# Voyager0587/yolov8-vit

Measured on AMD Instinct MI355X. Metric: images/sec end-to-end (640->224 detect+classify), higher is better.
Workload: dtype bf16; 1 GPU; YOLOv8n(nc=5)+ViT-B/16 end-to-end inference, 640x640, bf16 (BASELINE.json configs[1]); batch_per_gpu=32, global_batch=32, crops_per_image=4, parallelism=dp1, weights=random-init, seed 42

## Files before the change

### include/yv_hip.h

```cpp
#ifndef YV_HIP_H
#define YV_HIP_H

#include <stddef.h>
#include <stdint.h>

#ifdef __cplusplus
extern "C" {
#endif

#define YV_OK 0
#define YV_ERR_ARG (-1)
#define YV_ERR_LIMIT (-2)
#define YV_ERR_WORKSPACE (-3)
#define YV_ERR_LAUNCH (-4)

int yv_version(void);
const char* yv_error_string(int code);
int yv_device_is_gfx950(void);
int yv_set_option(const char* key, int value);
int yv_get_option(const char* key, int* value);

int yv_linear_mxfp8_q(const void* Aq, long long lda, const void* Ascale, long long a_rows_pad, const void* Wq, const void* Wscale,
                      long long w_rows_pad, const float* bias, int M, int N, int K, int flags, const int32_t* m_dev, int m_mul,
                      void* out_q, long long ldq, void* out_scales, long long out_rows_pad, void* stream);
// ... 102 lines not shown
    int ld;
    int c;
    int up;
} yv_view;

#define YV_EPI_BIAS 1
#define YV_EPI_SILU 2
#define YV_EPI_GELU 4
#define YV_EPI_RES_F32 8
#define YV_EPI_RES_BF16 16
#define YV_EPI_OUT_F32 32
#define YV_EPI_POSEMB 64
#define YV_EPI_SAVE_PRE 128
#define YV_EPI_GELU_BWD 256
#define YV_EPI_OUT_MXFP8 512

int yv_conv2d(const yv_view* in0, const yv_view* in1, int B, int Hout, int Wout, int ksize, int stride,
              const void* weight, const float* bias, int Cout, void* out, int out_ld, const void* res, int res_ld,
              int flags, void* stream);

int yv_conv2d_instance(int B, int Hout, int Wout, int ksize, int stride, int c0, int c1, int Cout, int out_ld, int res_ld,
                       int flags, size_t ws_bytes);

typedef struct yv_mx_view {
    const void* q;
    const void* s;
    int ld;
    int c;
    int up;
} yv_mx_view;

int yv_quant_mxfp8_map(const void* x, long long ldx, long long pixels, int C, void* q, long long ldq, void* scales,
                       void* stream);

int yv_conv2d_mxfp8(const yv_mx_view* in0, const yv_mx_view* in1, int B, int Hout, int Wout, int ksize, int stride,
                    const void* wq, const void* wscale, long long w_rows_pad, const float* bias, int Cout, void* out_bf16,
                    int out_ld, void* out_q, void* out_scales, int outq_ld, const void* res, int res_ld, int flags,
                    void* stream);
int yv_conv2d_mxfp8_instance(int B, int Hout, int Wout, int ksize, int stride, int Cin, int Cout);

int yv_c2f_fused(const void* x, long long ldx, int B, int H, int W, int c, int n, const void* w_cv1, const float* b_cv1,
                 const void* const* w_m, const float* const* b_m, const void* w_cv2, const float* b_cv2, void* out,
                 long long ldo, void* stream);
int yv_c2f_debug(void* buf);

int yv_conv2d_ws(const yv_view* in0, const yv_view* in1, int B, int Hout, int Wout, int ksize, int stride,
// ... 171 lines not shown
```

### yolov8-vit_amd/csrc/gemm.hip

```cpp
#include <string.h>
#include <type_traits>
#include <map>
#include <mutex>
#include "gemm_common.h"

using namespace yvgemm;

thread_local hipEvent_t yvgemm::t_time_start = nullptr, yvgemm::t_time_stop = nullptr;

namespace {

int g_opt_wgrad_split = 0;
int g_opt_wgrad_cap = 128;
int g_opt_variant = 1;
int g_opt_group_m = 8;
int g_opt_staged = 1;
int g_opt_p8 = 3;
std::mutex g_ws_mu;
std::map<void*, std::pair<void*, size_t>> g_ws;
static bool ws_lookup(void* stream, void** ws, size_t* bytes) {
    std::lock_guard<std::mutex> lk(g_ws_mu);
    auto it = g_ws.find(stream);
    if (it == g_ws.end()) return false;
    *ws = it->second.first; *bytes = it->second.second;
// ... 60 lines not shown
                float* o = (float*)g.out + orow * g.ldo + n;
                if (flags & YV_EPI_RES_F32) {
                    const float4 x = *(const float4*)o;
                    v[0] += x.x; v[1] += x.y; v[2] += x.z; v[3] += x.w;
                }
                *(float4*)o = make_float4(v[0], v[1], v[2], v[3]);
            } else {
                uint16_t* o = (uint16_t*)g.out + orow * g.ldo + n;
                *(uint2*)o = make_uint2(pack_bf16x2(v[0], v[1]), pack_bf16x2(v[2], v[3]));
                if constexpr (STATS) {
                    const uint32_t pk[2] = {pack_bf16x2(v[0], v[1]), pack_bf16x2(v[2], v[3])};
#pragma unroll
                    for (int q = 0; q < 4; ++q) {
                        const float f = bf16_to_f32((uint16_t)(q & 1 ? pk[q >> 1] >> 16 : pk[q >> 1] & 0xffff));
                        cs[i * 4 + q] += f; cq[i * 4 + q] += f * f;
                    }
                }
            }
        }
    }
}


template <int MF, bool STATS = false, bool PHASE = false >
__device__ __forceinline__ void epilogue_staged(const GemmArgs& g, f32x4 (&acc)[4][MF], int M, int m0, int n0,
                                                int wrow_m, int wrow_n, int lane, unsigned char* stage, float* cs = nullptr,
                                                float* cq = nullptr, int ph = 0) {
    const int flags = g.flags;
    const int fr = lane & 15, fq = lane >> 4;
    const int nb = n0 + wrow_n;
    float4 bv[4];
#pragma unroll
    for (int i = 0; i < 4; ++i) {
        const int n = nb + i * 16 + fq * 4;
        bv[i] = ((flags & YV_EPI_BIAS) && n < g.N) ? *(const float4*)(g.bias + n) : make_float4(0.f, 0.f, 0.f, 0.f);
    }
    auto value = [&](int i, int j, float* v, bool act = true) {
        v[0] = acc[i][j][0] + bv[i].x; v[1] = acc[i][j][1] + bv[i].y;
        v[2] = acc[i][j][2] + bv[i].z; v[3] = acc[i][j][3] + bv[i].w;
        if (!act) return;
        if (flags & YV_EPI_SILU) {
#pragma unroll
            for (int q = 0; q < 4; ++q) v[q] = silu_f(v[q]);
        }
        if (flags & YV_EPI_GELU) {
#pragma unroll
            for (int q = 0; q < 4; ++q) v[q] = gelu_f(v[q]);
        }
    };
    if (!(flags & (YV_EPI_OUT_F32 | YV_EPI_RES_F32))) {
        if (flags & YV_EPI_SAVE_PRE) {
#pragma unroll
            for (int j = 0; j < MF; ++j)
#pragma unroll
                for (int i = 0; i < 4; ++i) {
                    float v[4];
                    value(i, j, v, false);
                    const int row = j * 16 + fr, c16 = i * 2 + (fq >> 1);
                    *(uint2*)(stage + row * 128 + ((c16 ^ (row & 7)) << 4) + (fq & 1) * 8) =
                        make_uint2(pack_bf16x2(v[0], v[1]), pack_bf16x2(v[2], v[3]));
                }
#pragma unroll
            for (int it = 0; it < MF * 2; ++it) {
                const int row = it * 8 + (lane >> 3), ch = lane & 7;
                const int m = m0 + wrow_m + row, n = nb + ch * 8;
                const uint4 pk = *(const uint4*)(stage + row * 128 + ((ch ^ (row & 7)) << 4));
                if (m < M && n < g.N) *(uint4*)(g.aux + (long long)m * g.ldaux + n) = pk;
            }
        }
#pragma unroll
        for (int j = 0; j < MF; ++j)
#pragma unroll
            for (int i = 0; i < 4; ++i) {
                float v[4];
                value(i, j, v);
                const int row = j * 16 + fr, c16 = i * 2 + (fq >> 1);
                *(uint2*)(stage + row * 128 + ((c16 ^ (row & 7)) << 4) + (fq & 1) * 8) =
                    make_uint2(pack_bf16x2(v[0], v[1]), pack_bf16x2(v[2], v[3]));
            }
#pragma unroll
        for (int it = 0; it < MF * 2; ++it) {
            const int row = it * 8 + (lane >> 3), ch = lane & 7;
            const int m = m0 + wrow_m + row, n = nb + ch * 8;
            uint4 pk = *(const uint4*)(stage + row * 128 + ((ch ^ (row & 7)) << 4));
            if (m < M && n < g.N) {
                [[maybe_unused]] long long om = 0;
                if constexpr (PHASE) om = phase_row<true>(g, m, ph);
                if (flags & YV_EPI_RES_BF16) {
                    const uint4 rr = *(const uint4*)(g.res + (PHASE ? om : (long long)m) * g.ldres + n);
                    const uint32_t a[4] = {pk.x, pk.y, pk.z, pk.w}, b[4] = {rr.x, rr.y, rr.z, rr.w};
                    uint32_t o[4];
#pragma unroll
                    for (int q = 0; q < 4; ++q)
                        o[q] = pack_bf16x2(bf16_to_f32((uint16_t)(a[q] & 0xffff)) + bf16_to_f32((uint16_t)(b[q] & 0xffff)),
                                           bf16_to_f32((uint16_t)(a[q] >> 16)) + bf16_to_f32((uint16_t)(b[q] >> 16)));
                    pk = make_uint4(o[0], o[1], o[2], o[3]);
                }
                if (flags & YV_EPI_OUT_MXFP8) {
                    const uint32_t a[4] = {pk.x, pk.y, pk.z, pk.w};
                    float f[8];
#pragma unroll
                    for (int q = 0; q < 4; ++q) { f[2 * q] = bf16_to_f32((uint16_t)(a[q] & 0xffff)); f[2 * q + 1] = bf16_to_f32((uint16_t)(a[q] >> 16)); }
                    float amax = 0.f;
#pragma unroll
                    for (int q = 0; q < 8; ++q) amax = fmaxf(amax, fabsf(f[q]));
                    amax = fmaxf(amax, __shfl_xor(amax, 1, 64));
                    amax = fmaxf(amax, __shfl_xor(amax, 2, 64));
                    int e = -127;
                    if (amax > 0.f) {
                        int ex;
                        const float mant = frexpf(amax * (1.0f / 448.0f), &ex);
                        e = mant == 0.5f ? ex - 1 : ex;
                        e = e < -127 ? -127 : (e > 127 ? 127 : e);
                    }
                    const float inv = ldexpf(1.0f, -e);
                    int p0 = 0, p1 = 0;
                    p0 = __builtin_amdgcn_cvt_pk_fp8_f32(f[0] * inv, f[1] * inv, p0, false);
                    p0 = __builtin_amdgcn_cvt_pk_fp8_f32(f[2] * inv, f[3] * inv, p0, true);
                    p1 = __builtin_amdgcn_cvt_pk_fp8_f32(f[4] * inv, f[5] * inv, p1, false);
                    p1 = __builtin_amdgcn_cvt_pk_fp8_f32(f[6] * inv, f[7] * inv, p1, true);
                    *(uint2*)(g.mxq + (long long)m * g.ldmxq + n) = make_uint2((uint32_t)p0, (uint32_t)p1);
                    if ((ch & 3) == 0) {
                        const int bk = n >> 5;
                        g.mxs[((long long)(bk >> 2) * g.mx_rows + m) * 4 + (bk & 3)] = (uint8_t)(e + 127);
                    }
                    continue;
                }
                if (flags & YV_EPI_GELU_BWD) {
                    const uint4 uu = *(const uint4*)(g.aux + (long long)m * g.ldaux + n);
                    const uint32_t a[4] = {pk.x, pk.y, pk.z, pk.w}, b[4] = {uu.x, uu.y, uu.z, uu.w};
                    uint32_t o[4];
#pragma unroll
                    for (int q = 0; q < 4; ++q)
                        o[q] = pack_bf16x2(bf16_to_f32((uint16_t)(a[q] & 0xffff)) * gelu_grad_f(bf16_to_f32((uint16_t)(b[q] & 0xffff))),
                                           bf16_to_f32((uint16_t)(a[q] >> 16)) * gelu_grad_f(bf16_to_f32((uint16_t)(b[q] >> 16))));
                    pk = make_uint4(o[0], o[1], o[2], o[3]);
                }
                *(uint4*)((uint16_t*)g.out + (PHASE ? om : (long long)m) * g.ldo + n) = pk;
                if constexpr (STATS) {
                    const uint32_t a[4] = {pk.x, pk.y, pk.z, pk.w};
#pragma unroll
                    for (int q = 0; q < 8; ++q) {
                        const float f = bf16_to_f32((uint16_t)(q & 1 ? a[q >> 1] >> 16 : a[q >> 1] & 0xffff));
                        cs[q] += f; cq[q] += f * f;
                    }
                }
            }
        }
    } else {
#pragma unroll
        for (int half = 0; half < 2; ++half) {
#pragma unroll
            for (int jj = 0; jj < MF / 2; ++jj)
#pragma unroll
                for (int i = 0; i < 4; ++i) {
                    float v[4];
                    value(i, half * (MF / 2) + jj, v);
                    const int row = jj * 16 + fr, c16 = i * 4 + fq;
                    *(float4*)(stage + row * 256 + ((c16 ^ (row & 15)) << 4)) = make_float4(v[0], v[1], v[2], v[3]);
                }
#pragma unroll
            for (int it = 0; it < MF * 2; ++it) {
                const int row = it * 4 + (lane >> 4), ch = lane & 15;
                const int m = m0 + wrow_m + half * (MF * 8) + row, n = nb + ch * 4;
                float4 v = *(const float4*)(stage + row * 256 + ((ch ^ (row & 15)) << 4));
                if (m < M && n < g.N) {
                    long long orow = m;
                    if (flags & YV_EPI_POSEMB) {
                        const int r = m / g.tok, t = m - r * g.tok;
                        orow = (long long)r * (g.tok + 1) + 1 + t;
                        const float4 pp = *(const float4*)(g.pos + (long long)(1 + t) * g.N + n);
                        v.x += pp.x; v.y += pp.y; v.z += pp.z; v.w += pp.w;
// ... 666 lines not shown
            bf16x8 fa[MF], fw[NF];
            const int kc = ks * 4 + fq;
#pragma unroll
            for (int j = 0; j < MF; ++j) {
                const int rr = wrow_m + j * 16 + fr;
                fa[j] = *(const bf16x8*)(A + rr * 128 + ((kc ^ (rr & 7)) << 4));
            }
#pragma unroll
            for (int i = 0; i < NF; ++i) {
                const int rr = wrow_n + i * 16 + fr;
                fw[i] = *(const bf16x8*)(W + rr * 128 + ((kc ^ (rr & 7)) << 4));
            }
#pragma unroll
            for (int i = 0; i < NF; ++i)
#pragma unroll
                for (int j = 0; j < MF; ++j)
                    acc[i][j] = __builtin_amdgcn_mfma_f32_16x16x32_bf16(fw[i], fa[j], acc[i][j], 0, 0, 0);
        }
    }
    asm volatile("s_barrier" ::: "memory");
    finish_tile<MF, NF, STATS, WM, BN, PHASE>(g, acc, M, m0, n0, wrow_m, wrow_n, lane, wave, smem, tm, ph);
}


struct MxArgs {
    GemmArgs g;
    const uint8_t* sa;
    const uint8_t* sw;
    long long rows_a, rows_w;
};

template <int BM, int BN, int WM, int WN>
__global__ __launch_bounds__(WM * WN * 64) void gemm_mx_kernel(MxArgs a) {
    const GemmArgs& g = a.g;
    constexpr int NW = WM * WN, MF = BM / WM / 16, NF = BN / WN / 16, A_BYTES = BM * 128, W_BYTES = BN * 128;
    constexpr int A_INS = BM / (8 * NW), W_INS = BN / (8 * NW);
    constexpr int S_INS = (BM + BN + 255) / 256;
    constexpr int S_BYTES = S_INS * 1024;
    constexpr int STAGE = A_BYTES + W_BYTES + S_BYTES;
    extern __shared__ __attribute__((aligned(16))) unsigned char smem[];
    const int tid = threadIdx.x, lane = tid & 63, wave = tid >> 6;
    int M = g.M;
    if (g.m_dev) { long long md = (long long)g.m_dev[0] * g.m_mul; M = md < M ? (int)md : M; }
    int bid = blockIdx.x;
    {
        const int nwg = gridDim.x, q = nwg >> 3, r = nwg & 7, x = bid & 7;
// ... 993 lines not shown
    if (lds < (size_t)THREADS / 64 * (BM / WM) * 128) lds = (size_t)THREADS / 64 * (BM / WM) * 128;
    void (*kern)(GemmArgs) = igemm_kernel<MODE, BM, BN, WM, WN, false>;
    if constexpr (MODE == 1) { if (g.c1 > 0) kern = igemm_kernel<MODE, BM, BN, WM, WN, true>; }
    if constexpr (MODE == 1 && BM == 128) { if (g.stats) kern = igemm_kernel<MODE, BM, BN, WM, WN, false, true>; }
    if (!yv_grant_lds((const void*)kern, lds)) return YV_ERR_LAUNCH;
    const int S = g.splitk > 1 ? g.splitk : 1;
    hipLaunchKernelGGL(kern, dim3(g.tiles_m * g.tiles_n * S), dim3(THREADS), lds, st, g);
    return launch_splitk_reduce(g, st);
}


bool epi_can_stage(const GemmArgs& g) {
    const bool f32 = g.flags & (YV_EPI_OUT_F32 | YV_EPI_RES_F32);
    const int al = f32 ? 4 : 8;
    if ((g.N % al) || (g.ldo % al) || ((uintptr_t)g.out & 15)) return false;
    if ((g.flags & YV_EPI_RES_BF16) && ((g.ldres % 8) || ((uintptr_t)g.res & 15))) return false;
    if ((g.flags & (YV_EPI_SAVE_PRE | YV_EPI_GELU_BWD)) && ((g.ldaux % 8) || ((uintptr_t)g.aux & 15))) return false;
    return true;
}

int g_opt_dgrad_s2_split = 0;
int g_opt_conv_dma = 8;

template <int BN, int WM, int WN, int ST>
int launch_cdma(GemmArgs& g, hipStream_t st) {
    g.tiles_m = (g.M + 127) / 128;
    g.tiles_n = (g.N + BN - 1) / BN;
    const size_t lds = ST * (size_t)(128 + BN) * 128;
    void (*kern)(GemmArgs) = cgemm_dma_kernel<BN, WM, WN, ST>;
    if (g.stats) kern = cgemm_dma_kernel<BN, WM, WN, ST, true>;
    if (!yv_grant_lds((const void*)kern, lds)) return YV_ERR_LAUNCH;
    hipLaunchKernelGGL(kern, dim3(g.tiles_m * g.tiles_n), dim3(256), lds, st, g);
    return yv_launch_status();
}

template <int BN, int WM, int WN>
int launch_cmx(ConvMxArgs& a, hipStream_t st) {
    a.g.tiles_m = (a.g.M + 127) / 128;
    a.g.tiles_n = (a.g.N + BN - 1) / BN;
    auto kern = cgemm_mx_kernel<BN, WM, WN>;
    hipLaunchKernelGGL(kern, dim3(a.g.tiles_m * a.g.tiles_n), dim3(256), 2 * (128 + BN) * 128, st, a);
    return yv_launch_status();
}

enum ConvKern {
    CK_IGEMM_16 = 0, CK_IGEMM_32 = 1, CK_IGEMM_64 = 2, CK_IGEMM_128 = 3,
    CK_CDMA_64_2 = 4, CK_CDMA_64_3 = 5, CK_CDMA_64_4 = 6, CK_CDMA_128_2 = 7, CK_CDMA_128_3 = 8
};
// ... 23 lines not shown
        if (g_opt_conv_dma == 5)
            return g.K >= 1024 ? CK_CDMA_64_3 : two_stage;
        if (g_opt_conv_dma == 7)
            return g.M >= 100000 ? two_stage : CK_CDMA_64_3;
        if (g_opt_conv_dma == 8)
            return (g.M >= 100000 && g.N > 64) ? CK_CDMA_128_2 : CK_CDMA_64_3;
        if (g_opt_conv_dma == 6)
            return g.K >= 1024 ? CK_CDMA_64_3 : CK_CDMA_64_2;
        return two_stage;
    }
    return igemm_pick(g.N);
}

template <int MODE>
int launch_igemm(GemmArgs& g, int kern, hipStream_t st) {
    switch (kern) {
    case CK_IGEMM_128: return launch<MODE, 128, 128, 2, 2>(g, st);
    case CK_IGEMM_64: return launch<MODE, 128, 64, 4, 1>(g, st);
    case CK_IGEMM_32: return launch<MODE, 128, 32, 4, 1>(g, st);
    default: return launch<MODE, 128, 16, 4, 1>(g, st);
    }
}

int launch_conv(GemmArgs& g, int kern, hipStream_t st) {
    switch (kern) {
    case CK_CDMA_64_2: return launch_cdma<64, 4, 1, 2>(g, st);
    case CK_CDMA_64_3: return launch_cdma<64, 4, 1, 3>(g, st);
    case CK_CDMA_64_4: return launch_cdma<64, 4, 1, 4>(g, st);
    case CK_CDMA_128_2: return launch_cdma<128, 2, 2, 2>(g, st);
    case CK_CDMA_128_3: return launch_cdma<128, 2, 2, 3>(g, st);
    default: return launch_igemm<1>(g, kern, st);
    }
}

int launch_phases(void (*kern)(GemmArgs), GemmArgs& g, int threads, size_t lds, hipStream_t st) {
    const int per = g.tiles_m * g.tiles_n;
    if (!g_opt_dgrad_s2_split) {
        g.group_m = 0;
        hipLaunchKernelGGL(kern, dim3(4 * per), dim3(threads), lds, st, g);
        return yv_launch_status();
    }
    for (int q = 0; q < 4; ++q) {
        g.group_m = q;
        hipLaunchKernelGGL(kern, dim3(per), dim3(threads), lds, st, g);
        const int rc = yv_launch_status();
        if (rc != YV_OK) return rc;
    }
    return YV_OK;
}

template <int BN, int WM, int WN>
int launch_phase_igemm(GemmArgs& g, hipStream_t st) {
    g.tiles_m = (g.M + 127) / 128;
// ... 360 lines not shown
extern "C" int yv_set_launch_timing(void* start_event, void* stop_event) {
    t_time_start = (hipEvent_t)start_event;
    t_time_stop = (hipEvent_t)stop_event;
    return YV_OK;
}

static const struct { const char* key; int* (*at)(); } k_options[] = {
    {"linear_variant", [] { return &g_opt_variant; }},
    {"wgrad_split_cap", [] { return &g_opt_wgrad_cap; }},
    {"wgrad_split", [] { return &g_opt_wgrad_split; }},
    {"linear_p9_small", [] { return &g_opt_p9_small; }},
    {"linear_p9_small_fixed", [] { return &g_opt_p9_small_fixed; }},
    {"linear_group_m", [] { return &g_opt_group_m; }},
    {"staged_epilogue", [] { return &g_opt_staged; }},
    {"linear_p8", [] { return &g_opt_p8; }},
    {"linear_p8_rows", [] { return &g_opt_p8_rows; }},
    {"linear_p8_cus", [] { return &g_opt_p8_cus; }},
    {"linear_p8_sched", [] { return &g_opt_p8_sched; }},
    {"conv_splitk", [] { return &g_opt_splitk; }},
    {"linear_splitk", [] { return &g_opt_linear_splitk; }},
    {"linear_skinny", [] { return &g_opt_skinny; }},
    {"wgrad_mx_split", [] { return &g_opt_wgrad_mx_split; }},
    {"conv_dma", [] { return &g_opt_conv_dma; }},
    {"dgrad_s2_split", [] { return &g_opt_dgrad_s2_split; }},
};
static int* option_at(const char* key) {
    for (const auto& o : k_options)
        if (key && !strcmp(key, o.key)) return o.at();
    return nullptr;
}

extern "C" int yv_set_option(const char* key, int value) {
    int* const opt = option_at(key);
    if (!opt) return YV_ERR_ARG;
    *opt = value;
    return YV_OK;
}

extern "C" int yv_get_option(const char* key, int* value) {
    const int* const opt = option_at(key);
    if (!opt || !value) return YV_ERR_ARG;
    *value = *opt;
    return YV_OK;
}

static int launch_linear(GemmArgs& g, const LinearRoute& r, void* ws, int n_cu, hipStream_t st) {
// ... 65 lines not shown
                       (hipStream_t)stream);
}

extern "C" int yv_linear_route(int M, int N, int K, int lda, int ldo, int flags, int has_res_f32, int ldaux, int mx, size_t ws_bytes,
                               int n_cu, yv_linear_route_t* out) {
    static unsigned char dummy[16] __attribute__((aligned(16)));
    if (!out || M <= 0 || n_cu < 0) return YV_ERR_ARG;
    const LinearQuery q = {out, ws_bytes, persistent_cus(n_cu)};
    const float* f = (const float*)dummy;
    const int32_t* m_dev = (flags & YV_ROUTE_M_DEV) ? (const int32_t*)dummy : nullptr;
    flags &= ~YV_ROUTE_M_DEV;
    if (!mx)
        return linear_impl(dummy, lda, dummy, f, M, N, K, dummy, ldo, f, 1, flags, m_dev, 1, has_res_f32 ? f : nullptr,
                           ldaux > 0 ? dummy : nullptr, ldaux, nullptr, &q);
    if (flags & YV_EPI_OUT_MXFP8) return YV_ERR_ARG;
    return linear_mx_impl(dummy, lda, dummy, (M + 127) / 128 * 128LL, dummy, dummy, (N + 127) / 128 * 128LL, f, M, N, K, dummy, ldo,
                          flags, m_dev, 1, nullptr, 0, nullptr, 0, nullptr, has_res_f32 ? f : nullptr, ldaux > 0 ? dummy : nullptr,
                          ldaux, &q);
}

static int conv_impl_one(const yv_view* in0, const yv_view* in1, int B, int Hout, int Wout, int ksize, int stride,
                         const void* weight, const float* bias, int Cout, void* out, int out_ld, const void* res,
                         int res_ld, int flags, void* ws, size_t ws_bytes, void* stream, bool query = false,
                         float* stats = nullptr ) {
    if (!in0 || !in0->ptr || !weight || !out || B <= 0 || Hout <= 0 || Wout <= 0 || Cout <= 0) return YV_ERR_ARG;
    if (!(ksize == 1 || ksize == 3) || !(stride == 1 || stride == 2)) return YV_ERR_ARG;
    if (in1 && in1->ptr && ksize != 1) return YV_ERR_ARG;
    const int c1 = (in1 && in1->ptr) ? in1->c : 0;
    const int Cin = in0->c + c1;
    if ((in0->c & 7) || (c1 & 7) || (in0->ld & 7) || (c1 && (in1->ld & 7)) || (Cout & 3) || (out_ld & 3))
        return YV_ERR_ARG;
    if ((flags & YV_EPI_BIAS) && !bias) return YV_ERR_ARG;
    if ((flags & YV_EPI_RES_BF16) && (!res || (res_ld & 3))) return YV_ERR_ARG;
    if (flags & (YV_EPI_GELU | YV_EPI_POSEMB | YV_EPI_RES_F32)) return YV_ERR_ARG;
    if ((long long)B * Hout * Wout > 0x7fffffffLL) return YV_ERR_LIMIT;
    if (ksize == 3 && in0->up) return YV_ERR_ARG;
    {
        const long long px = (long long)B * Hout * stride * Wout * stride;
        if ((px + Wout * stride + 1) * in0->ld * 2 >= 0x7fffffffLL || (c1 && px * in1->ld * 2 >= 0x7fffffffLL) ||
            (long long)Cout * ksize * ksize * Cin * 2 >= 0x7fffffffLL)
            return YV_ERR_LIMIT;
    }
    GemmArgs g = {};
    g.cin_shift = (Cin & (Cin - 1)) == 0 ? __builtin_ctz((unsigned)Cin) : -1;
    g.tap_uniform = (Cin % 64) == 0;
    g.a0 = (const uint16_t*)in0->ptr; g.lda0 = in0->ld; g.c0 = in0->c; g.up0 = in0->up;
    if (c1) { g.a1 = (const uint16_t*)in1->ptr; g.lda1 = in1->ld; g.c1 = c1; g.up1 = in1->up; }
    g.Hin = Hout * stride; g.Win = Wout * stride;
    g.Hout = Hout; g.Wout = Wout; g.ksize = ksize; g.stride = stride;
    g.w = (const uint16_t*)weight; g.bias = bias;
    g.M = B * Hout * Wout; g.N = Cout; g.K = ksize * ksize * Cin;
    g.out = out; g.ldo = out_ld; g.res = (const uint16_t*)res; g.ldres = res_ld; g.flags = flags;
    const int kern = conv_route(g, ws != nullptr && !stats, ws_bytes);
    if (query) return conv_instance_code(g, kern);
    if (g.splitk > 1) g.partial = (float*)ws;
    g.stats = stats;
    return launch_conv(g, kern, (hipStream_t)stream);
}

static int conv_impl(const yv_view* in0, const yv_view* in1, int B, int Hout, int Wout, int ksize, int stride,
                     const void* weight, const float* bias, int Cout, void* out, int out_ld, const void* res,
                     int res_ld, int flags, void* ws, size_t ws_bytes, void* stream, bool query = false) {
    if (!in0 || !in0->ptr || B <= 0 || Hout <= 0 || Wout <= 0 || !out)
        return conv_impl_one(in0, in1, B, Hout, Wout, ksize, stride, weight, bias, Cout, out, out_ld, res, res_ld, flags, ws, ws_bytes,
                             stream, query);
    const long long Hin = (long long)Hout * stride, Win = (long long)Wout * stride;
    const bool two = in1 && in1->ptr;
    const long long s0 = (Hin >> in0->up) * (Win >> in0->up) * in0->ld * 2;
    const long long s1 = two ? (Hin >> in1->up) * (Win >> in1->up) * in1->ld * 2 : 0;
    const long long nb = conv_sub_batch(s0, s1, (Win + 1) * in0->ld * 2);
    if (nb >= B)
        return conv_impl_one(in0, in1, B, Hout, Wout, ksize, stride, weight, bias, Cout, out, out_ld, res, res_ld, flags, ws, ws_bytes,
                             stream, query);
    if (nb < 1) return YV_ERR_LIMIT;
    const long long esz = (flags & YV_EPI_OUT_F32) ? 4 : 2;
    for (long long b0 = 0; b0 < B; b0 += nb) {
        const int n = (int)(B - b0 < nb ? B - b0 : nb);
        yv_view v0 = *in0, v1 = two ? *in1 : yv_view{};
        v0.ptr = (unsigned char*)in0->ptr + b0 * s0;
        if (two) v1.ptr = (unsigned char*)in1->ptr + b0 * s1;
        const int rc = conv_impl_one(&v0, two ? &v1 : nullptr, n, Hout, Wout, ksize, stride, weight, bias, Cout,
                                     (unsigned char*)out + b0 * Hout * Wout * out_ld * esz, out_ld,
                                     res ? (const unsigned char*)res + b0 * Hout * Wout * res_ld * 2 : nullptr, res_ld, flags, ws, ws_bytes,
                                     stream, query);
        if (rc != YV_OK || query) return rc;
    }
    return YV_OK;
}

extern "C" int yv_linear_nn(const void* A, int lda, const void* Wkn, int ldw, const float* bias, int M, int N, int K,
                            void* out, int ldo, int flags, void* aux, int ldaux, void* stream) {
    if (!A || !Wkn || !out || M <= 0 || N <= 0 || K <= 0) return YV_ERR_ARG;
    if ((K % BK) || (lda & 7) || (ldw & 7) || (N & 7) || (ldo & 7)) return YV_ERR_ARG;
    if (flags & ~(YV_EPI_BIAS | YV_EPI_GELU_BWD)) return YV_ERR_ARG;
    if ((flags & YV_EPI_BIAS) && !bias) return YV_ERR_ARG;
    if ((flags & YV_EPI_GELU_BWD) && !aux) return YV_ERR_ARG;
    if (((uintptr_t)A | (uintptr_t)Wkn | (uintptr_t)out) & 15) return YV_ERR_ARG;
    GemmArgs g = {};
    g.a0 = (const uint16_t*)A; g.lda0 = lda; g.c0 = K;
    g.w = (const uint16_t*)Wkn; g.ldw = ldw; g.bias = bias; g.M = M; g.N = N; g.K = K;
    g.out = out; g.ldo = ldo; g.flags = flags; g.aux = (uint16_t*)aux; g.ldaux = ldaux;
    g.ksize = 1; g.stride = 1; g.splitk = 1;
    g.staged = epi_can_stage(g);
    if (!g.staged) return YV_ERR_ARG;
    g.group_m = g_opt_group_m > 0 ? g_opt_group_m : 8;
    return launch_dma<128, 128, 2, 2, 0, true>(g, (hipStream_t)stream);
}
// ... 94 lines not shown
                               const float* bias, int Cout, void* out, int out_ld, int flags, float* stats_ws, size_t stats_ws_floats,
                               void* ws, size_t ws_bytes, void* stream) {
    if (!stats_ws || (flags & ~YV_EPI_BIAS) || Cout <= 0 || (Cout & 7)) return YV_ERR_ARG;
    const int code = conv_impl_one(in0, nullptr, B, Hout, Wout, ksize, stride, weight, bias, Cout, out, out_ld, nullptr, 0, flags, ws,
                                   ws_bytes, stream, true, stats_ws);
    if (code < 0) return code;
    {
        const long long Hin = (long long)Hout * stride, Win = (long long)Wout * stride;
        const long long s0 = (Hin >> in0->up) * (Win >> in0->up) * in0->ld * 2;
        if (conv_sub_batch(s0, 0, (Win + 1) * in0->ld * 2) < B) return YV_ERR_LIMIT;
    }
    if (stats_ws_floats < yv_conv_stats_ws_floats((long long)B * Hout * Wout, Cout)) return YV_ERR_WORKSPACE;
    return conv_impl_one(in0, nullptr, B, Hout, Wout, ksize, stride, weight, bias, Cout, out, out_ld, nullptr, 0, flags, ws, ws_bytes,
                         stream, false, stats_ws);
}

extern "C" int yv_conv2d_instance(int B, int Hout, int Wout, int ksize, int stride, int c0, int c1, int Cout, int out_ld,
                                  int res_ld, int flags, size_t ws_bytes) {
    static unsigned char dummy[16] __attribute__((aligned(16)));
    if (c0 <= 0 || c1 < 0) return YV_ERR_ARG;
    const yv_view v0 = {dummy, c0, c0, 0}, v1 = {dummy, c1, c1, 0};
    return conv_impl(&v0, c1 ? &v1 : nullptr, B, Hout, Wout, ksize, stride, dummy, (const float*)dummy, Cout, dummy, out_ld,
                     (flags & YV_EPI_RES_BF16) ? dummy : nullptr, res_ld, flags, ws_bytes ? dummy : nullptr, ws_bytes, nullptr, true);
}

static int dgrad_s2_one(const yv_view* dz, int B, int Hout, int Wout, const void* wd, int Cin, int Cout, void* dx, int dx_ld,
                        const void* res, int res_ld, void* stream, yv_dgrad_s2_route_t* route) {
    GemmArgs g = {};
    g.cin_shift = (Cout & (Cout - 1)) == 0 ? __builtin_ctz((unsigned)Cout) : -1;
    g.tap_uniform = 1;
    g.a0 = (const uint16_t*)dz->ptr; g.lda0 = dz->ld; g.c0 = Cout;
    g.Hin = Hout; g.Win = Wout; g.Hout = Hout; g.Wout = Wout; g.ksize = 3; g.stride = 1;
    g.w = (const uint16_t*)wd;
    g.M = B * Hout * Wout; g.N = Cin; g.K = 9 * Cout;
    g.out = dx; g.ldo = dx_ld; g.res = (const uint16_t*)res; g.ldres = res_ld; g.flags = res ? YV_EPI_RES_BF16 : 0;
    const int kern = dgrad_s2_route(g);
    if (route) {
        const int bn = kern == CK_CDMA_128_2 || kern == CK_IGEMM_128 ? 128 : (kern == CK_IGEMM_32 ? 32 : (kern == CK_IGEMM_16 ? 16 : 64));
        route->kernel = kern;
        route->staged = g.staged && kern >= CK_IGEMM_64;
        for (int q = 0; q < 4; ++q) route->ksteps[q] = (q == 0 ? 4 : (q == 3 ? 1 : 2)) * (Cout / BK);
        route->tiles = ((g.M + 127) / 128) * ((g.N + bn - 1) / bn);
        route->workgroups = 4 * route->tiles;
        route->use = 1;
        return YV_OK;
    }
// ... 157 lines not shown
```

### yolov8-vit_amd/yvhip/__init__.py

```python
from __future__ import annotations

import collections
import ctypes as C
import os

_HWQ_PRESET = os.environ.get("GPU_MAX_HW_QUEUES")
os.environ.setdefault("GPU_MAX_HW_QUEUES", "8")
import re
from typing import List, Optional, Tuple

import torch

HW_QUEUES = int(_HWQ_PRESET) if _HWQ_PRESET else (4 if torch.cuda.is_initialized() else 8)

_HERE = os.path.dirname(os.path.abspath(__file__))
LIB_PATH = os.path.join(_HERE, "libyvhip.so")
HEADER_PATH = os.path.normpath(os.path.join(_HERE, "..", "..", "include", "yv_hip.h"))


class YvError(RuntimeError):
    pass


def _load():
# ... 65 lines not shown
    "yv_c2f_fused": (_i, [_vp, C.c_longlong, _i, _i, _i, _i, _i, _vp, _vp, _vp, _vp, _vp, _vp, _vp, C.c_longlong, _vp]),
    "yv_optim_step": (_i, [_i, _vp, _vp, _vp, _vp, _sz, _f, _f, _f, _f, _f, _f, _i, _vp, _vp]),
    "yv_ema_update": (_i, [_vp, _vp, _sz, _f, _vp]),
    "yv_axpby": (_i, [_vp, _vp, _sz, _f, _f, _vp]),
    "yv_detect_loss_ws_bytes": (_sz, [_i, _i, _i]),
    "yv_detect_loss": (_i, [_vp, _vp, _vp, _vp, _i, _i, _i, _i, _vp, _vp, _vp, _i, _f, _f, _f, _vp, _vp, _sz, _vp]),
    "yv_blob_nhwc8": (_i, [_vp, C.c_longlong, _vp, _vp]),
    "yv_bn_ws_floats": (_sz, [C.c_longlong, _i]),
    "yv_bn_stats": (_i, [_vp, C.c_longlong, C.c_longlong, _i, _f, _f, _vp, _vp, _vp, _vp, _vp, _sz, _vp]),
    "yv_bn_stats_finish": (_i, [_vp, C.c_longlong, _i, _f, _f, _vp, _vp, _vp, _vp, _vp]),
    "yv_conv_stats_ws_floats": (_sz, [C.c_longlong, _i]),
    "yv_conv2d_stats": (_i, [C.POINTER(yv_view), _i, _i, _i, _i, _i, _vp, _vp, _i, _vp, _i, _i, _vp, _sz, _vp, _sz, _vp]),
    "yv_bn_act_fwd": (_i, [_vp, C.c_longlong, C.c_longlong, _i, _vp, _vp, _vp, _vp, _vp, C.c_longlong, _vp, C.c_longlong,
                           _i, _vp]),
    "yv_bn_act_bwd": (_i, [_vp, C.c_longlong, _vp, C.c_longlong, C.c_longlong, _i, _vp, _vp, _vp, _vp, _i, _i, _vp, _vp,
                           _vp, C.c_longlong, _vp, _sz, _vp]),
    "yv_view_op": (_i, [_i, _vp, C.c_longlong, _vp, C.c_longlong, _i, _i, _i, _i, _vp]),
    "yv_maxpool5_bwd": (_i, [_vp, C.c_longlong, _vp, C.c_longlong, _vp, C.c_longlong, _i, _i, _i, _i, _vp, _sz, _vp]),
    "yv_im2col3": (_i, [_vp, C.c_longlong, _i, _i, _i, _i, _i, _vp, _vp]),
    "yv_conv_weight_dgrad": (_i, [_vp, _i, _i, _i, _vp, _vp]),
    "yv_conv2d": (_i, [C.POINTER(yv_view), C.POINTER(yv_view), _i, _i, _i, _i, _i, _vp, _vp, _i, _vp, _i, _vp, _i,
                       _i, _vp]),
    "yv_conv2d_instance": (_i, [_i, _i, _i, _i, _i, _i, _i, _i, _i, _i, _i, _sz]),
    "yv_conv2d_dgrad_s2": (_i, [C.POINTER(yv_view), _i, _i, _i, _vp, _i, _i, _vp, _i, _vp, _i, _vp, _sz, _vp]),
    "yv_conv2d_dgrad_s2_route": (_i, [_i, _i, _i, _i, _i, _i, _i, _i, _i, _vp]),
    "yv_conv2d_ws": (_i, [C.POINTER(yv_view), C.POINTER(yv_view), _i, _i, _i, _i, _i, _vp, _vp, _i, _vp, _i, _vp, _i,
                          _i, _vp, _sz, _vp]),
    "yv_linear": (_i, [_vp, _i, _vp, _vp, _i, _i, _i, _vp, _i, _vp, _i, _i, _vp, _i, _vp]),
    "yv_layernorm": (_i, [_vp, _sz, _vp, _vp, _i, _i, _f, _vp, _sz, _vp, _i, _vp]),
    "yv_linear_res_ln": (_i, [_vp, _i, _vp, _vp, _i, _i, _i, _vp, _i, _vp, _vp, _f, _vp, _i, _vp, _i, _vp]),
    "yv_attention": (_i, [_vp, _i, _i, _i, _f, _vp, _vp, _vp]),
    "yv_attention_cls": (_i, [_vp, _vp, _i, _i, _i, _f, _vp, _vp, _vp]),
    "yv_attention_long": (_i, [_vp, _i, _i, _i, _f, _vp, _vp, _vp, _vp, C.c_longlong, _vp, C.c_longlong, _vp]),
    "yv_attention_debug": (_i, [_i]),
    "yv_cls_rows": (_i, [_vp, _vp, _i, _i, _i, _vp, _vp]),
    "yv_wrapper_head": (_i, [_vp, _i, _vp, _vp, _vp, _vp, _i, _i, _f, _i, _vp, _vp, _vp, _vp]),
    "yv_sppf_pool": (_i, [_vp, _i, _i, _i, _i, _i, _vp]),
    "yv_stem_conv": (_i, [_vp, _i, _i, _i, _vp, _vp, _i, _vp, _i, _vp]),
    "yv_linear_ex": (_i, [_vp, _i, _vp, _vp, _i, _i, _i, _vp, _i, _i, _vp, _vp, _i, _vp]),
    "yv_attention_train": (_i, [_vp, _i, _i, _i, _f, _vp, _vp, _vp]),
    "yv_attention_bwd": (_i, [_vp, _vp, _vp, _vp, _i, _i, _i, _f, _vp, _vp, _vp]),
    "yv_attention_bwd_long": (_i, [_vp, _vp, _vp, _vp, _i, _i, _i, _f, _vp, _vp, _vp]),
    "yv_attention_bwd_short": (_i, [_vp, _vp, _vp, _vp, _i, _i, _i, _f, _vp, _vp, _vp]),
    "yv_attention_cls_train": (_i, [_vp, C.c_longlong, _vp, _i, _i, _i, _f, _vp, _vp, _vp]),
    "yv_attention_cls_bwd": (_i, [_vp, C.c_longlong, _vp, _vp, _vp, _i, _i, _i, _f, _vp, _vp]),
    "yv_linear_nn": (_i, [_vp, _i, _vp, _i, _vp, _i, _i, _i, _vp, _i, _i, _vp, _i, _vp]),
# ... 507 lines not shown
    optr = C.c_void_p(out.data_ptr() + esz * out_c_off)
    rptr = None if res is None else C.c_void_p(res.data_ptr() + 2 * res_c_off)
    ws = _conv_workspace(out.device)
    check(lib.yv_conv2d_ws(C.byref(in0), C.byref(in1) if in1 is not None else None, B, Hout, Wout, ksize, stride,
                           _p(weight), _p(bias), Cout, optr, out.shape[-1], rptr,
                           0 if res is None else res.shape[-1], flags | EPI_BIAS, _p(ws), ws.numel() * 4, _st()),
          "yv_conv2d_ws")
    return out


CONV_WS_BYTES = 16 * 1024 * 1024 * 4
CONV_IGEMM_16, CONV_IGEMM_32, CONV_IGEMM_64, CONV_IGEMM_128 = 0, 1, 2, 3
CONV_DMA_64_2, CONV_DMA_64_3, CONV_DMA_64_4, CONV_DMA_128_2, CONV_DMA_128_3 = 4, 5, 6, 7, 8
CONV_STAGED, CONV_SPLITK, CONV_TWO = 16, 32, 64


def conv2d_instance(B: int, Hout: int, Wout: int, ksize: int, stride: int, c0: int, c1: int, Cout: int, out_ld: int,
                    res_ld: int = 0, flags: int = 0, ws_bytes: int = CONV_WS_BYTES) -> int:
    r = lib.yv_conv2d_instance(B, Hout, Wout, ksize, stride, c0, c1, Cout, out_ld, res_ld, flags | EPI_BIAS, ws_bytes)
    check(min(r, 0), "yv_conv2d_instance")
    return r


def layernorm(x: torch.Tensor, gamma: torch.Tensor, beta: torch.Tensor, y: torch.Tensor, rows: int, D: int,
              ldx: int, ldy: int, eps: float = 1e-6, count_dev: Optional[torch.Tensor] = None,
              rows_per_count: int = 1):
    check(lib.yv_layernorm(_p(x), ldx, _p(gamma), _p(beta), rows, D, float(eps), _p(y), ldy, _p(count_dev),
                           rows_per_count, _st()), "yv_layernorm")
    return y


def attention(qkv: torch.Tensor, R: int, N: int, H: int, out: torch.Tensor, scale: Optional[float] = None,
              r_dev: Optional[torch.Tensor] = None):
    _chk_dev(qkv, out, r_dev)
    check(lib.yv_attention(_p(qkv), R, N, H, float(64 ** -0.5 if scale is None else scale), _p(out), _p(r_dev),
                           _st()), "yv_attention")
    return out


def attention_long(qkv: torch.Tensor, R: int, N: int, H: int, out: Optional[torch.Tensor] = None, scale: Optional[float] = None,
                   r_dev: Optional[torch.Tensor] = None, lse: Optional[torch.Tensor] = None,
                   out_q: Optional[torch.Tensor] = None, out_scale: Optional[torch.Tensor] = None):
    _chk_dev(qkv, out, r_dev, lse, out_q, out_scale)
    if (out_q is None) != (out_scale is None):
        raise YvError("attention_long: out_q and out_scale come together")
    check(lib.yv_attention_long(_p(qkv), R, N, H, float(64 ** -0.5 if scale is None else scale), _p(out), _p(r_dev), _p(lse),
# ... 607 lines not shown
```

Baseline: 4785 images/s.

## Add halo-tiled 3x3 stride-1 conv kernel that stages input tile once in LDS

Adds a new implicit-GEMM conv kernel for 3x3 stride-1 convolutions. It loads an 8x16 output tile plus a one-pixel halo of input for all channels into LDS once, then walks the nine taps by shifting row offsets into that buffer, so input is not re-fetched for every kernel position. Only weights are streamed through a multi-stage ring. The staged epilogue gains a halo row-mapping mode, and a heuristic picks halo or the old path based on LDS size and padding waste. The costs are larger LDS use, which can lower occupancy, and wasted work on partially filled edge tiles.

```diff
diff --git a/include/yv_hip.h b/include/yv_hip.h
--- a/include/yv_hip.h
+++ b/include/yv_hip.h
@@ -148,6 +148,18 @@
 int yv_conv2d_instance(int B, int Hout, int Wout, int ksize, int stride, int c0, int c1, int Cout, int out_ld, int res_ld,
                        int flags, size_t ws_bytes);
 
+enum {
+    YV_HALO_ON = 0,
+    YV_HALO_OPTION = 1,
+    YV_HALO_ROUTE = 2,
+    YV_HALO_SHAPE = 3,
+    YV_HALO_FORM = 4,
+    YV_HALO_LDS = 5,
+    YV_HALO_SLOWER = 6
+};
+int yv_conv2d_halo(int B, int Hout, int Wout, int ksize, int stride, int c0, int in_ld, int c1, int Cout, int out_ld, int res_ld,
+                   int flags, int stats, size_t ws_bytes);
+
 typedef struct yv_mx_view {
     const void* q;
     const void* s;
diff --git a/yolov8-vit_amd/csrc/gemm.hip b/yolov8-vit_amd/csrc/gemm.hip
--- a/yolov8-vit_amd/csrc/gemm.hip
+++ b/yolov8-vit_amd/csrc/gemm.hip
@@ -106,10 +106,12 @@
 }
 
 
-template <int MF, bool STATS = false, bool PHASE = false >
+template <int MF, bool STATS = false, int RM = 0>
 __device__ __forceinline__ void epilogue_staged(const GemmArgs& g, f32x4 (&acc)[4][MF], int M, int m0, int n0,
                                                 int wrow_m, int wrow_n, int lane, unsigned char* stage, float* cs = nullptr,
-                                                float* cq = nullptr, int ph = 0) {
+                                                float* cq = nullptr, int ph = 0, int lim = 0) {
+    constexpr bool PHASE = RM == 1, HALO = RM == 2;
+    static_assert(!(HALO && STATS), "no column sums on the halo body");
     const int flags = g.flags;
     const int fr = lane & 15, fq = lane >> 4;
     const int nb = n0 + wrow_n;
@@ -133,7 +135,7 @@
         }
     };
     if (!(flags & (YV_EPI_OUT_F32 | YV_EPI_RES_F32))) {
-        if (flags & YV_EPI_SAVE_PRE) {
+        if (!HALO && (flags & YV_EPI_SAVE_PRE)) {
 #pragma unroll
             for (int j = 0; j < MF; ++j)
 #pragma unroll
@@ -167,11 +169,14 @@
             const int row = it * 8 + (lane >> 3), ch = lane & 7;
             const int m = m0 + wrow_m + row, n = nb + ch * 8;
             uint4 pk = *(const uint4*)(stage + row * 128 + ((ch ^ (row & 7)) << 4));
-            if (m < M && n < g.N) {
+            bool in = m < M;
+            if constexpr (HALO) in = (m >> 4) < (lim >> 8) && (m & 15) < (lim & 255);
+            if (in && n < g.N) {
                 [[maybe_unused]] long long om = 0;
                 if constexpr (PHASE) om = phase_row<true>(g, m, ph);
+                if constexpr (HALO) om = (long long)ph + (m >> 4) * g.Wout + (m & 15);
                 if (flags & YV_EPI_RES_BF16) {
-                    const uint4 rr = *(const uint4*)(g.res + (PHASE ? om : (long long)m) * g.ldres + n);
+                    const uint4 rr = *(const uint4*)(g.res + (RM ? om : (long long)m) * g.ldres + n);
                     const uint32_t a[4] = {pk.x, pk.y, pk.z, pk.w}, b[4] = {rr.x, rr.y, rr.z, rr.w};
                     uint32_t o[4];
 #pragma unroll
@@ -180,7 +185,7 @@
                                            bf16_to_f32((uint16_t)(a[q] >> 16)) + bf16_to_f32((uint16_t)(b[q] >> 16)));
                     pk = make_uint4(o[0], o[1], o[2], o[3]);
                 }
-                if (flags & YV_EPI_OUT_MXFP8) {
+                if (!HALO && (flags & YV_EPI_OUT_MXFP8)) {
                     const uint32_t a[4] = {pk.x, pk.y, pk.z, pk.w};
                     float f[8];
 #pragma unroll
@@ -210,7 +215,7 @@
                     }
                     continue;
                 }
-                if (flags & YV_EPI_GELU_BWD) {
+                if (!HALO && (flags & YV_EPI_GELU_BWD)) {
                     const uint4 uu = *(const uint4*)(g.aux + (long long)m * g.ldaux + n);
                     const uint32_t a[4] = {pk.x, pk.y, pk.z, pk.w}, b[4] = {uu.x, uu.y, uu.z, uu.w};
                     uint32_t o[4];
@@ -220,7 +225,7 @@
                                            bf16_to_f32((uint16_t)(a[q] >> 16)) * gelu_grad_f(bf16_to_f32((uint16_t)(b[q] >> 16))));
                     pk = make_uint4(o[0], o[1], o[2], o[3]);
                 }
-                *(uint4*)((uint16_t*)g.out + (PHASE ? om : (long long)m) * g.ldo + n) = pk;
+                *(uint4*)((uint16_t*)g.out + (RM ? om : (long long)m) * g.ldo + n) = pk;
                 if constexpr (STATS) {
                     const uint32_t a[4] = {pk.x, pk.y, pk.z, pk.w};
 #pragma unroll
@@ -231,7 +236,7 @@
                 }
             }
         }
-    } else {
+    } else if constexpr (!HALO) {
 #pragma unroll
         for (int half = 0; half < 2; ++half) {
 #pragma unroll
@@ -944,6 +949,122 @@
     finish_tile<MF, NF, STATS, WM, BN, PHASE>(g, acc, M, m0, n0, wrow_m, wrow_n, lane, wave, smem, tm, ph);
 }
 
+constexpr int HALO_TH = 8, HALO_TW = 16, HALO_PW = HALO_TW + 2, HALO_PIX = (HALO_TH + 2) * HALO_PW;
+constexpr int HALO_PIECES = (HALO_PIX + 7) / 8;
+constexpr int HALO_SLICE = HALO_PIECES * 1024;
+
+template <int BN, int WM, int WN, int ST>
+__global__ __launch_bounds__(256) void cgemm_halo_kernel(GemmArgs g) {
+    constexpr int NW = 4;
+    static_assert(WM * WN == NW, "four waves");
+    constexpr int MF = 128 / WM / 16, NF = BN / WN / 16;
+    static_assert(NF == 4 && (MF % 2) == 0, "the staged epilogue's wave tile");
+    constexpr int W_BYTES = BN * 128, W_INS = BN / (8 * NW);
+    extern __shared__ __attribute__((aligned(16))) unsigned char smem[];
+    const int tid = threadIdx.x, lane = tid & 63, wave = __builtin_amdgcn_readfirstlane(tid >> 6);
+    int bid = blockIdx.x;
+    {
+        const int nwg = gridDim.x, q = nwg >> 3, r = nwg & 7, x = bid & 7;
+        bid = (x < r ? x * (q + 1) : r * (q + 1) + (x - r) * q) + (bid >> 3);
+    }
+    const int tm = bid / g.tiles_n, tn = bid - tm * g.tiles_n;
+    const int n0 = tn * BN;
+    const int H = g.Hout, Wd = g.Wout;
+    const int TX = (Wd + HALO_TW - 1) / HALO_TW, TY = (H + HALO_TH - 1) / HALO_TH;
+    const int b = tm / (TX * TY), trem = tm - b * (TX * TY);
+    const int y0 = (trem / TX) * HALO_TH, x0 = (trem % TX) * HALO_TW;
+
+    const int lrow = lane >> 3, lch = lane & 7;
+    constexpr uint32_t OOB = 0x80000000u;
+    const int nslice = g.c0 >> 6;
+    const auto rs0 = __builtin_amdgcn_make_buffer_rsrc((void*)g.a0, 0, 0x7fffffff, 0x00020000);
+    const auto rsW = __builtin_amdgcn_make_buffer_rsrc((void*)g.w, 0, 0x7fffffff, 0x00020000);
+    for (int q = wave; q < HALO_PIECES; q += NW) {
+        const int p = q * 8 + lrow;
+        const int py = p / HALO_PW, px = p - py * HALO_PW;
+        const int iy = y0 + py - 1, ix = x0 + px - 1;
+        const bool ok = p < HALO_PIX && iy >= 0 && iy < H && ix >= 0 && ix < Wd;
+        const uint32_t off = ok ? (uint32_t)((((long long)b * H + iy) * Wd + ix) * g.lda0 * 2) + (uint32_t)((lch ^ lrow) << 4) : OOB;
+        for (int s = 0; s < nslice; ++s)
+            __builtin_amdgcn_raw_ptr_buffer_load_lds(rs0, (lptr_t)(smem + s * HALO_SLICE + q * 1024), 16, (int)off, s * 128, 0, 0);
+    }
+    unsigned char* const ring = smem + nslice * HALO_SLICE;
+    uint32_t w_off[W_INS];
+#pragma unroll
+    for (int j = 0; j < W_INS; ++j) {
+        const int r = (j * NW + wave) * 8 + lrow;
+        int n = n0 + r;
+        n = n < g.N ? n : g.N - 1;
+        w_off[j] = (uint32_t)(((long long)n * g.K + ((lch ^ (r & 7)) << 3)) * 2);
+    }
+    auto issue = [&](int kt, int buf) __attribute__((always_inline)) {
+        unsigned char* W = ring + buf * W_BYTES;
+#pragma unroll
+        for (int j = 0; j < W_INS; ++j)
+            __builtin_amdgcn_raw_ptr_buffer_load_lds(rsW, (lptr_t)(W + (j * NW + wave) * 1024), 16, (int)w_off[j], kt * BK * 2, 0, 0);
+    };
+
+    f32x4 acc[NF][MF];
+#pragma unroll
+    for (int i = 0; i < NF; ++i)
+#pragma unroll
+        for (int j = 0; j < MF; ++j) acc[i][j] = (f32x4){0.f, 0.f, 0.f, 0.f};
+    const int wm = wave / WN, wn = wave - wm * WN;
+    const int wrow_m = wm * (128 / WM), wrow_n = wn * (BN / WN);
+    const int fr = lane & 15, fq = lane >> 4;
+    const int prow0 = (wrow_m >> 4) * HALO_PW + fr;
+    const int nk = g.K / BK;
+    int issued = 0;
+#pragma unroll
+    for (int p = 0; p < ST - 1; ++p)
+        if (p < nk) { issue(p, p); ++issued; }
+    int slot = 0, islot = (ST - 1) % ST;
+    int sl = 0, disp = 0, kx = 0;
+    for (int kt = 0; kt < nk; ++kt) {
+        if (issued - kt - 1 >= ST - 2 && ST > 2) {
+            if constexpr (ST == 3) asm volatile("s_waitcnt vmcnt(%0)" :: "n"(W_INS) : "memory");
+            else if constexpr (ST == 4) asm volatile("s_waitcnt vmcnt(%0)" :: "n"(2 * W_INS) : "memory");
+            else asm volatile("s_waitcnt vmcnt(0)" ::: "memory");
+        } else {
+            asm volatile("s_waitcnt vmcnt(0)" ::: "memory");
+        }
+        asm volatile("s_barrier" ::: "memory");
+        __builtin_amdgcn_sched_barrier(0);
+        if (issued < nk) { issue(issued, islot); ++issued; islot = islot + 1 == ST ? 0 : islot + 1; }
+        const unsigned char* A = smem + sl * HALO_SLICE;
+        const unsigned char* W = ring + slot * W_BYTES;
+        slot = slot + 1 == ST ? 0 : slot + 1;
+#pragma unroll
+        for (int ks = 0; ks < 2; ++ks) {
+            bf16x8 fa[MF], fw[NF];
+            const int kc = ks * 4 + fq;
+#pragma unroll
+            for (int j = 0; j < MF; ++j) {
+                const int rr = prow0 + j * HALO_PW + disp;
+                fa[j] = *(const bf16x8*)(A + rr * 128 + ((kc ^ (rr & 7)) << 4));
+            }
+#pragma unroll
+            for (int i = 0; i < NF; ++i) {
+                const int rr = wrow_n + i * 16 + fr;
+                fw[i] = *(const bf16x8*)(W + rr * 128 + ((kc ^ (rr & 7)) << 4));
+            }
+#pragma unroll
+            for (int i = 0; i < NF; ++i)
+#pragma unroll
+                for (int j = 0; j < MF; ++j)
+                    acc[i][j] = __builtin_amdgcn_mfma_f32_16x16x32_bf16(fw[i], fa[j], acc[i][j], 0, 0, 0);
+        }
+        if (++sl == nslice) {
+            sl = 0;
+            if (++kx == 3) { kx = 0; disp += HALO_PW - 2; } else ++disp;
+        }
+    }
+    asm volatile("s_barrier" ::: "memory");
+    const int vy = H - y0 < HALO_TH ? H - y0 : HALO_TH, vx = Wd - x0 < HALO_TW ? Wd - x0 : HALO_TW;
+    epilogue_staged<MF, false, 2>(g, acc, 128, 0, n0, wrow_m, wrow_n, lane, smem + wave * (MF * 16 * 128), nullptr, nullptr,
+                                  (b * H + y0) * Wd + x0, (vy << 8) | vx);
+}
+
 
 struct MxArgs {
     GemmArgs g;
@@ -1983,8 +2104,25 @@
 int g_opt_dgrad_s2_split = 0;
 int g_opt_conv_dma = 8;
 
+int g_opt_conv_halo = 1;
+
+size_t conv_halo_lds(int Cin, int BN, int ST) { return (size_t)(Cin / 64) * HALO_SLICE + (size_t)ST * BN * 128; }
+
 template <int BN, int WM, int WN, int ST>
-int launch_cdma(GemmArgs& g, hipStream_t st) {
+int launch_chalo(GemmArgs& g, hipStream_t st) {
+    const int TX = (g.Wout + HALO_TW - 1) / HALO_TW, TY = (g.Hout + HALO_TH - 1) / HALO_TH;
+    g.tiles_m = (g.M / (g.Hout * g.Wout)) * TX * TY;
+    g.tiles_n = (g.N + BN - 1) / BN;
+    const size_t lds = conv_halo_lds(g.c0, BN, ST);
+    void (*kern)(GemmArgs) = cgemm_halo_kernel<BN, WM, WN, ST>;
+    if (!yv_grant_lds((const void*)kern, lds)) return YV_ERR_LAUNCH;
+    hipLaunchKernelGGL(kern, dim3(g.tiles_m * g.tiles_n), dim3(256), lds, st, g);
+    return yv_launch_status();
+}
+
+template <int BN, int WM, int WN, int ST>
+int launch_cdma(GemmArgs& g, hipStream_t st, bool halo) {
+    if (halo) return launch_chalo<BN, WM, WN, ST>(g, st);
     g.tiles_m = (g.M + 127) / 128;
     g.tiles_n = (g.N + BN - 1) / BN;
     const size_t lds = ST * (size_t)(128 + BN) * 128;
@@ -2054,13 +2192,34 @@
     }
 }
 
-int launch_conv(GemmArgs& g, int kern, hipStream_t st) {
+bool conv_halo_slower(const GemmArgs& g, int BN, int ST) {
+    const int tiles_n = (g.N + BN - 1) / BN;
+    if (2 * conv_halo_lds(g.c0, BN, ST) > 160 * 1024 && tiles_n >= 2) return true;
+    const long long per_image = (long long)((g.Hout + HALO_TH - 1) / HALO_TH) * ((g.Wout + HALO_TW - 1) / HALO_TW);
+    const long long images = g.M / ((long long)g.Hout * g.Wout);
+    const bool padded = per_image * 128 * 2 >= (long long)g.Hout * g.Wout * 3;
+    return padded && images * per_image * tiles_n > 512;
+}
+
+int conv_halo_reason(const GemmArgs& g, int kern, bool stats, bool sub) {
+    if (!g_opt_conv_halo) return YV_HALO_OPTION;
+    if (kern < CK_CDMA_64_2 || kern > CK_CDMA_128_3) return YV_HALO_ROUTE;
+    if (g.ksize != 3 || g.stride != 1 || g.c1) return YV_HALO_SHAPE;
+    if (stats || sub) return YV_HALO_FORM;
+    if (g.flags & ~(YV_EPI_BIAS | YV_EPI_SILU | YV_EPI_RES_BF16)) return YV_HALO_FORM;
+    const int BN = kern >= CK_CDMA_128_2 ? 128 : 64, ST = kern == CK_CDMA_64_4 ? 4 : (kern == CK_CDMA_64_2 || kern == CK_CDMA_128_2 ? 2 : 3);
+    if (conv_halo_lds(g.c0, BN, ST) > 160 * 1024) return YV_HALO_LDS;
+    if (g_opt_conv_halo == 2) return YV_HALO_ON;
+    return conv_halo_slower(g, BN, ST) ? YV_HALO_SLOWER : YV_HALO_ON;
+}
+
+int launch_conv(GemmArgs& g, int kern, hipStream_t st, bool halo = false) {
     switch (kern) {
-    case CK_CDMA_64_2: return launch_cdma<64, 4, 1, 2>(g, st);
-    case CK_CDMA_64_3: return launch_cdma<64, 4, 1, 3>(g, st);
-    case CK_CDMA_64_4: return launch_cdma<64, 4, 1, 4>(g, st);
-    case CK_CDMA_128_2: return launch_cdma<128, 2, 2, 2>(g, st);
-    case CK_CDMA_128_3: return launch_cdma<128, 2, 2, 3>(g, st);
+    case CK_CDMA_64_2: return launch_cdma<64, 4, 1, 2>(g, st, halo);
+    case CK_CDMA_64_3: return launch_cdma<64, 4, 1, 3>(g, st, halo);
+    case CK_CDMA_64_4: return launch_cdma<64, 4, 1, 4>(g, st, halo);
+    case CK_CDMA_128_2: return launch_cdma<128, 2, 2, 2>(g, st, halo);
+    case CK_CDMA_128_3: return launch_cdma<128, 2, 2, 3>(g, st, halo);
     default: return launch_igemm<1>(g, kern, st);
     }
 }
@@ -2467,6 +2626,7 @@
     {"linear_skinny", [] { return &g_opt_skinny; }},
     {"wgrad_mx_split", [] { return &g_opt_wgrad_mx_split; }},
     {"conv_dma", [] { return &g_opt_conv_dma; }},
+    {"conv_halo", [] { return &g_opt_conv_halo; }},
     {"dgrad_s2_split", [] { return &g_opt_dgrad_s2_split; }},
 };
 static int* option_at(const char* key) {
@@ -2578,7 +2738,8 @@
 static int conv_impl_one(const yv_view* in0, const yv_view* in1, int B, int Hout, int Wout, int ksize, int stride,
                          const void* weight, const float* bias, int Cout, void* out, int out_ld, const void* res,
                          int res_ld, int flags, void* ws, size_t ws_bytes, void* stream, bool query = false,
-                         float* stats = nullptr ) {
+                         float* stats = nullptr ,
+                         bool sub = false , int* halo = nullptr ) {
     if (!in0 || !in0->ptr || !weight || !out || B <= 0 || Hout <= 0 || Wout <= 0 || Cout <= 0) return YV_ERR_ARG;
     if (!(ksize == 1 || ksize == 3) || !(stride == 1 || stride == 2)) return YV_ERR_ARG;
     if (in1 && in1->ptr && ksize != 1) return YV_ERR_ARG;
@@ -2608,18 +2769,22 @@
     g.M = B * Hout * Wout; g.N = Cout; g.K = ksize * ksize * Cin;
     g.out = out; g.ldo = out_ld; g.res = (const uint16_t*)res; g.ldres = res_ld; g.flags = flags;
     const int kern = conv_route(g, ws != nullptr && !stats, ws_bytes);
-    if (query) return conv_instance_code(g, kern);
+    const int halo_why = conv_halo_reason(g, kern, stats != nullptr, sub);
+    if (query) {
+        if (halo) *halo = halo_why;
+        return conv_instance_code(g, kern);
+    }
     if (g.splitk > 1) g.partial = (float*)ws;
     g.stats = stats;
-    return launch_conv(g, kern, (hipStream_t)stream);
+    return launch_conv(g, kern, (hipStream_t)stream, halo_why == YV_HALO_ON);
 }
 
 static int conv_impl(const yv_view* in0, const yv_view* in1, int B, int Hout, int Wout, int ksize, int stride,
                      const void* weight, const float* bias, int Cout, void* out, int out_ld, const void* res,
-                     int res_ld, int flags, void* ws, size_t ws_bytes, void* stream, bool query = false) {
+                     int res_ld, int flags, void* ws, size_t ws_bytes, void* stream, bool query = false, int* halo = nullptr) {
     if (!in0 || !in0->ptr || B <= 0 || Hout <= 0 || Wout <= 0 || !out)
         return conv_impl_one(in0, in1, B, Hout, Wout, ksize, stride, weight, bias, Cout, out, out_ld, res, res_ld, flags, ws, ws_bytes,
-                             stream, query);
+                             stream, query, nullptr, false, halo);
     const long long Hin = (long long)Hout * stride, Win = (long long)Wout * stride;
     const bool two = in1 && in1->ptr;
     const long long s0 = (Hin >> in0->up) * (Win >> in0->up) * in0->ld * 2;
@@ -2627,7 +2792,7 @@
     const long long nb = conv_sub_batch(s0, s1, (Win + 1) * in0->ld * 2);
     if (nb >= B)
         return conv_impl_one(in0, in1, B, Hout, Wout, ksize, stride, weight, bias, Cout, out, out_ld, res, res_ld, flags, ws, ws_bytes,
-                             stream, query);
+                             stream, query, nullptr, false, halo);
     if (nb < 1) return YV_ERR_LIMIT;
     const long long esz = (flags & YV_EPI_OUT_F32) ? 4 : 2;
     for (long long b0 = 0; b0 < B; b0 += nb) {
@@ -2638,7 +2803,7 @@
         const int rc = conv_impl_one(&v0, two ? &v1 : nullptr, n, Hout, Wout, ksize, stride, weight, bias, Cout,
                                      (unsigned char*)out + b0 * Hout * Wout * out_ld * esz, out_ld,
                                      res ? (const unsigned char*)res + b0 * Hout * Wout * res_ld * 2 : nullptr, res_ld, flags, ws, ws_bytes,
-                                     stream, query);
+                                     stream, query, nullptr, true, halo);
         if (rc != YV_OK || query) return rc;
     }
     return YV_OK;
@@ -2779,6 +2944,25 @@
     const yv_view v0 = {dummy, c0, c0, 0}, v1 = {dummy, c1, c1, 0};
     return conv_impl(&v0, c1 ? &v1 : nullptr, B, Hout, Wout, ksize, stride, dummy, (const float*)dummy, Cout, dummy, out_ld,
                      (flags & YV_EPI_RES_BF16) ? dummy : nullptr, res_ld, flags, ws_bytes ? dummy : nullptr, ws_bytes, nullptr, true);
+}
+
+extern "C" int yv_conv2d_halo(int B, int Hout, int Wout, int ksize, int stride, int c0, int in_ld, int c1, int Cout, int out_ld,
+                              int res_ld, int flags, int stats, size_t ws_bytes) {
+    static unsigned char dummy[16] __attribute__((aligned(16)));
+    if (c0 <= 0 || c1 < 0 || in_ld < c0) return YV_ERR_ARG;
+    const yv_view v0 = {dummy, in_ld, c0, 0}, v1 = {dummy, c1, c1, 0};
+    int why = YV_HALO_ROUTE;
+    int rc;
+    if (stats) {
+        if ((flags & ~YV_EPI_BIAS) || Cout <= 0 || (Cout & 7)) return YV_ERR_ARG;
+        rc = conv_impl_one(&v0, nullptr, B, Hout, Wout, ksize, stride, dummy, (const float*)dummy, Cout, dummy, out_ld, nullptr, 0,
+                           flags, ws_bytes ? dummy : nullptr, ws_bytes, nullptr, true, (float*)dummy, false, &why);
+    } else {
+        rc = conv_impl(&v0, c1 ? &v1 : nullptr, B, Hout, Wout, ksize, stride, dummy, (const float*)dummy, Cout, dummy, out_ld,
+                       (flags & YV_EPI_RES_BF16) ? dummy : nullptr, res_ld, flags, ws_bytes ? dummy : nullptr, ws_bytes, nullptr, true,
+                       &why);
+    }
+    return rc < 0 ? rc : why;
 }
 
 static int dgrad_s2_one(const yv_view* dz, int B, int Hout, int Wout, const void* wd, int Cin, int Cout, void* dx, int dx_ld,
diff --git a/yolov8-vit_amd/yvhip/__init__.py b/yolov8-vit_amd/yvhip/__init__.py
--- a/yolov8-vit_amd/yvhip/__init__.py
+++ b/yolov8-vit_amd/yvhip/__init__.py
@@ -111,6 +111,7 @@
     "yv_conv2d": (_i, [C.POINTER(yv_view), C.POINTER(yv_view), _i, _i, _i, _i, _i, _vp, _vp, _i, _vp, _i, _vp, _i,
                        _i, _vp]),
     "yv_conv2d_instance": (_i, [_i, _i, _i, _i, _i, _i, _i, _i, _i, _i, _i, _sz]),
+    "yv_conv2d_halo": (_i, [_i, _i, _i, _i, _i, _i, _i, _i, _i, _i, _i, _i, _i, _sz]),
     "yv_conv2d_dgrad_s2": (_i, [C.POINTER(yv_view), _i, _i, _i, _vp, _i, _i, _vp, _i, _vp, _i, _vp, _sz, _vp]),
     "yv_conv2d_dgrad_s2_route": (_i, [_i, _i, _i, _i, _i, _i, _i, _i, _i, _vp]),
     "yv_conv2d_ws": (_i, [C.POINTER(yv_view), C.POINTER(yv_view), _i, _i, _i, _i, _i, _vp, _vp, _i, _vp, _i, _vp, _i,
@@ -664,6 +665,18 @@
     return r
 
 
+HALO_ON, HALO_OPTION, HALO_ROUTE, HALO_SHAPE, HALO_FORM, HALO_LDS, HALO_SLOWER = 0, 1, 2, 3, 4, 5, 6
+
+
+def conv2d_halo(B: int, Hout: int, Wout: int, ksize: int, stride: int, c0: int, c1: int, Cout: int, out_ld: int,
+                res_ld: int = 0, flags: int = 0, ws_bytes: int = CONV_WS_BYTES, in_ld: Optional[int] = None,
+                stats: bool = False) -> int:
+    r = lib.yv_conv2d_halo(B, Hout, Wout, ksize, stride, c0, c0 if in_ld is None else in_ld, c1, Cout, out_ld, res_ld,
+                           flags | EPI_BIAS, int(stats), ws_bytes)
+    check(min(r, 0), "yv_conv2d_halo")
+    return r
+
+
 def layernorm(x: torch.Tensor, gamma: torch.Tensor, beta: torch.Tensor, y: torch.Tensor, rows: int, D: int,
               ldx: int, ldy: int, eps: float = 1e-6, count_dev: Optional[torch.Tensor] = None,
               rows_per_count: int = 1):
```

Result: no change. 4779 images/s (-0.1%).
